# LIA-DiTella/DiffUDF

Measured on AMD Instinct MI355X. Metric: train points/sec (SIREN fwd+∇x+Eikonal loss+bwd), 256×8 net, 100k pts, higher is better.
Workload: dtype f32

## Files before the change

### diffudf_amd/csrc/dudf_api.hip

```cpp
#include "dudf_context.h"

namespace {

int split_mask() { return dudf_split_mask(dudf_options()); }

int check_ws(const DudfLayout& lo, const void* ws, size_t bytes) {
    if (int rc = dudf_check_buffer(ws, bytes, lo.total_bytes)) return rc;
    if (lo.np > (1ll << 25)) return DUDF_E_BADCFG;
    return 0;
}

SweepRequest make_request(int which, int H, const SweepArgs& a) {
    return SweepRequest{which, H, a.L, a.store_s, a.store_c, a.train, a.have_e, a.split, a.p24, a.ebound != nullptr, a.zbound != nullptr};
}

int check_loss_mode(int mode, bool backward, int64_t n_hess, const double* weights, const double* stats) {
    if (mode != DUDF_LOSS_S1 && mode != DUDF_LOSS_SIREN && !(backward && mode == DUDF_LOSS_S2)) return DUDF_E_BADMODE;
    if (mode == DUDF_LOSS_S2 && !stats) return DUDF_E_BADMODE;
    if (n_hess != 0 && !(mode == DUDF_LOSS_S1 && weights[2] != 0.0)) return DUDF_E_BADMODE;
    return 0;
}

int64_t stash_offset(const DudfLayout& lo, int which) {
    const int64_t offs[8] = {lo.ws_S, lo.ws_C, lo.ws_Q, lo.ws_E, lo.ws_A, lo.ws_Z, lo.ws_R, lo.ws_ZS};
    return offs[which];
}

}

SweepArgs dudf_make_sweep_args(const DudfLayout& lo, const float* theta, float* ws) {
    SweepArgs a;
    a.theta = theta; a.w1b = ws + lo.ws_w1b; a.b1s = ws + lo.ws_b1s; a.w1t16 = ws + lo.ws_w1t16; a.wt = ws + lo.ws_wt;
    a.wimg_f = reinterpret_cast<const char*>(ws + lo.ws_wimg);
    a.wimg_t = a.wimg_f + (size_t)(lo.L - 1) * lo.H * lo.H * 6;
    a.wimg16_f = reinterpret_cast<const char*>(ws + lo.ws_wimg16);
    a.wimg16_t = a.wimg16_f + (size_t)(lo.L - 1) * lo.H * lo.H * 4;
    a.wsc = ws + lo.ws_wsc;
    a.amax = reinterpret_cast<unsigned*>(ws + lo.ws_amax);
    a.ebound = (lo.ws_ebound != lo.ws_amax) ? ws + lo.ws_ebound : nullptr;
    a.zbound = (lo.ws_zbound != lo.ws_amax) ? ws + lo.ws_zbound : nullptr;
    a.nch = lo.ncol_h;
    a.split = split_mask();
    a.clk = nullptr;
    a.x4 = ws + lo.ws_x4; a.y = ws + lo.ws_y; a.g = ws + lo.ws_g; a.ybar = ws + lo.ws_ybar; a.gbar = ws + lo.ws_gbar;
    a.S = ws + lo.ws_S; a.C = ws + lo.ws_C; a.ZS = ws + lo.ws_ZS; a.Q = ws + lo.ws_Q; a.R = ws + lo.ws_R;
    a.E = ws + lo.ws_E; a.A = ws + lo.ws_A; a.Z = ws + lo.ws_Z;
    a.np = lo.np; a.stash_layer = lo.stash_layer;
    a.off_hid = lo.off_hid; a.hid_stride = lo.hid_stride; a.off_wo = lo.off_wo; a.off_bo = lo.off_bo;
    a.L = lo.L; a.w0 = lo.w0;
    a.store_s = 0; a.store_c = 0; a.train = 0; a.have_e = 1;
    a.tile0 = 0; a.ntiles = 0; a.hess = 0;
    a.p24 = lo.p24;
    a.fxs = nullptr;
    return a;
}

int dudf_launch_range(int which, int H, SweepArgs a, hipStream_t st) {
    const SweepChoice c = dudf_choose_sweep(make_request(which, H, a), dudf_options());
    if (c.status) return c.status;
    DudfProfScope prof(PROF_SWEEP_FWD + (which & 3), st);
    if (which <= SWEEP_ADJ_REV) dudf_note_products(PROF_SWEEP_FWD + which, c.products);
    a.store_s = c.store_s; a.store_c = c.store_c;
    if (c.family == DUDF_FAM_F32) return dudf_launch_sweep(c, a, st);
    if (which <= SWEEP_ADJ_REV) a.clk = dudf_prof_clk(PROF_SWEEP_FWD + which);
    return dudf_launch_sweep_bf16(c, a, st);
}

int dudf_run_sweep(int base, const DudfLayout& lo, SweepArgs a, hipStream_t st) {
    int rc = 0;
    if ((lo.p24 & 1) && base >= SWEEP_FWD && base <= SWEEP_ADJ_REV) a.fxs = a.S - lo.ws_S + lo.ws_fx[base];
    SweepArgs aq = a, ap = a;
    aq.tile0 = 0; aq.ntiles = (int)(lo.ncol_h / DUDF_TILE_PTS); aq.hess = 1;
    ap.tile0 = aq.ntiles; ap.ntiles = (int)(lo.ncol_n / DUDF_TILE_PTS); ap.hess = 0;
    if (lo.ncol_h > 0 && lo.ncol_n > 0) {
        const SweepChoice c = dudf_choose_pair(make_request(base, lo.H, a), dudf_options());
        if (c.status == 0) {
            DudfProfScope prof(PROF_SWEEP_FWD + base, st);
            dudf_note_products(PROF_SWEEP_FWD + base, c.products);
            ap.clk = dudf_prof_clk(PROF_SWEEP_FWD + base);
            return dudf_launch_sweep_pair(c, aq, ap, st);
        }
    }
    if (lo.ncol_h > 0 && (rc = dudf_launch_range(base + 4, lo.H, aq, st))) return rc;
    if (lo.ncol_n > 0 && (rc = dudf_launch_range(base, lo.H, ap, st))) return rc;
    return 0;
}

int dudf_open_ctx(const dudf_net_cfg* cfg, int64_t n, int64_t n_h, void* workspace, size_t bytes, void* stream, DudfCtx* c,
                  int query_only) {
    int rc = dudf_make_layout(cfg, n, n_h, &c->lo, query_only);
    if (rc) return rc;
    if ((rc = check_ws(c->lo, workspace, bytes))) return rc;
    c->st = reinterpret_cast<hipStream_t>(stream);
    c->ws = reinterpret_cast<float*>(workspace);
    return 0;
}

int dudf_forward_common(DudfCtx& c, const float* theta, const float* x, int train, bool reverse) {
    int rc;
    const DudfLayout& lo = c.lo;
    const bool all16 = train && lo.ncol_h == 0 && dudf_use_bf16_sweeps() && (split_mask() & 15) == 15 && lo.L <= 32;
    const int need = (all16 ? 0 : 1) | (!dudf_use_bf16_sweeps() ? 2 : 0);
    rc = (lo.L >= 2) ? dudf_launch_prep(lo, theta, x, c.ws, need, c.st) : DUDF_E_UNSUPPORTED;
    if (rc == DUDF_E_UNSUPPORTED) {
        if ((rc = dudf_launch_pack(c.lo, theta, c.ws, c.st))) return rc;
        if (dudf_use_bf16_sweeps() && (rc = dudf_launch_pack_bf16(c.lo, theta, c.ws, c.st))) return rc;
        if (x && (rc = dudf_launch_make_x4(c.lo, x, c.ws, c.st))) return rc;
        hipError_t e = hipMemsetAsync(c.ws + c.lo.ws_acc, 0, (size_t)2 * DUDF_NACC * sizeof(float), c.st);
        if (e == hipSuccess) e = hipMemsetAsync(c.ws + c.lo.ws_amax, 0, (size_t)4 * c.lo.L * sizeof(unsigned), c.st);
        if (e != hipSuccess) return (int)e;
    } else if (rc) {
        return rc;
    }
    SweepArgs a = dudf_make_sweep_args(c.lo, theta, c.ws);
    a.store_s = train ? 1 : 0; a.store_c = (reverse || train) ? 1 : 0; a.train = train;
    if ((rc = dudf_run_sweep(SWEEP_FWD, c.lo, a, c.st))) return rc;
    if (reverse && (rc = dudf_run_sweep(SWEEP_REV, c.lo, a, c.st))) return rc;
    return 0;
}

int dudf_backward_common(DudfCtx& c, const float* theta, int have_g, float* dtheta, int accumulate, bool zeroed) {
    int rc;
    if (!accumulate && !zeroed) {
        hipError_t e = hipMemsetAsync(dtheta, 0, (size_t)c.lo.n_theta * sizeof(float), c.st);
        if (e != hipSuccess) return (int)e;
    }
    if ((rc = dudf_backward_sweeps(c, theta, have_g, zeroed))) return rc;
    return dudf_launch_wgrad(c.lo, c.ws, dtheta, have_g, c.st);
}

int dudf_backward_sweeps(DudfCtx& c, const float* theta, int have_g, bool zeroed) {
    int rc;
    SweepArgs a = dudf_make_sweep_args(c.lo, theta, c.ws);
    a.train = 1;
    if (dudf_split_fp16() && !(zeroed && 2 * c.lo.L <= 256)) {
        hipError_t e = hipMemsetAsync(c.ws + c.lo.ws_amax + c.lo.L, 0, (size_t)2 * c.lo.L * sizeof(unsigned), c.st);
        if (e != hipSuccess) return (int)e;
    }
    if (have_g) {
        if ((rc = dudf_run_sweep(SWEEP_ADJ_FWD, c.lo, a, c.st))) return rc;
    } else {
        a.have_e = 0;
    }
    return dudf_run_sweep(SWEEP_ADJ_REV, c.lo, a, c.st);
}

extern "C" {

int dudf_sweeps_bf16x6(const dudf_net_cfg* cfg) {
    if (!cfg) return 0;
    const SweepRequest r = {SWEEP_FWD, cfg->hidden, cfg->n_hidden_layers, 0, 0, 0, 1, split_mask(), 0, false, false};
    const SweepChoice c = dudf_choose_sweep(r, dudf_options());
    return (c.status == 0 && c.family != DUDF_FAM_F32) ? 1 : 0;
}

int64_t dudf_theta_count(const dudf_net_cfg* cfg) {
    DudfLayout lo;
    if (dudf_make_layout(cfg, 1, 0, &lo)) return -1;
    return lo.n_theta;
}

size_t dudf_workspace_bytes(const dudf_net_cfg* cfg, int64_t n) { return dudf_workspace_bytes_hess(cfg, n, 0); }

size_t dudf_workspace_bytes_query(const dudf_net_cfg* cfg, int64_t n, int64_t n_hess) {
    DudfLayout lo;
    if (dudf_make_layout(cfg, n, n_hess, &lo, 1)) return 0;
    return lo.total_bytes;
}

size_t dudf_workspace_bytes_hess(const dudf_net_cfg* cfg, int64_t n, int64_t n_hess) {
    DudfLayout lo;
    if (dudf_make_layout(cfg, n, n_hess, &lo)) return 0;
    return lo.total_bytes;
}

int dudf_stash_mode(const dudf_net_cfg* cfg, int64_t n, int64_t n_hess) {
    DudfLayout lo;
    if (dudf_make_layout(cfg, n, n_hess, &lo)) return -1;
    return lo.p24;
}

int dudf_loss_forward(const dudf_net_cfg* cfg, int mode, const float* theta, const float* x, const float* normals,
                      const float* sdf, int64_t n_local, int64_t n_global, int64_t n_hess, const double* weights,
                      double alpha, float* out_terms, void* workspace, size_t workspace_bytes, void* stream) {
    int rc = check_loss_mode(mode, false, n_hess, weights, nullptr);
    if (rc) return rc;
    DudfCtx c;
    if ((rc = dudf_open_ctx(cfg, n_local, n_hess, workspace, workspace_bytes, stream, &c))) return rc;
    if ((rc = dudf_forward_common(c, theta, x, 1, true))) return rc;
    return dudf_launch_loss_fwd(c.lo, mode, normals, sdf, n_global, weights, alpha, c.ws, out_terms, c.st);
}
// ... 154 lines not shown
```

### diffudf_amd/csrc/dudf_internal.h

```cpp
#pragma once
#include <hip/hip_runtime.h>
#include <stdint.h>
#include <stdlib.h>
#include "../../include/dudf_hip.h"
#include "dudf_variants.h"

typedef float f32x4 __attribute__((ext_vector_type(4)));
typedef float f32x16 __attribute__((ext_vector_type(16)));
typedef float f32x2 __attribute__((ext_vector_type(2)));
typedef unsigned u32x4 __attribute__((ext_vector_type(4)));
typedef __bf16 bf16x8 __attribute__((ext_vector_type(8)));
typedef __bf16 bf16x2 __attribute__((ext_vector_type(2)));
typedef _Float16 f16x8 __attribute__((ext_vector_type(8)));
typedef _Float16 f16x2 __attribute__((ext_vector_type(2)));

__device__ __forceinline__ unsigned cvt_pk(f32x2 v) {
    return __builtin_bit_cast(unsigned, __builtin_convertvector(v, bf16x2));
}
__device__ __forceinline__ f32x2 unpack(unsigned p) {
    return f32x2{__builtin_bit_cast(float, p << 16), __builtin_bit_cast(float, p & 0xffff0000u)};
}

#define DUDF_TILE_PTS 64
#define DUDF_COL_PAD 128
#define DUDF_NACC 16

struct DudfLayout {
    int H, L;
    float rho;
    int p24;
    float w0;
    int64_t n, n_h;
    int64_t ncol_h, ncol_n;
    int64_t ncols;
    int64_t np;
    int64_t off_w1, off_b1, off_hid, hid_stride, off_wo, off_bo, n_theta;
    int64_t ws_w1b, ws_b1s, ws_w1t16, ws_wt, ws_wimg, ws_wimg16, ws_wsc, ws_amax, ws_ebound, ws_zbound, ws_x4, ws_y, ws_g, ws_ybar, ws_gbar;
    int64_t ws_S, ws_C, ws_ZS, ws_Q, ws_R, ws_E, ws_A, ws_Z, ws_acc;
    int64_t ws_fx[4];
    int64_t stash_layer;
    size_t total_bytes;
};

DudfOptions dudf_options();
inline bool dudf_deterministic() { return dudf_options().deterministic != 0; }
inline bool dudf_split_fp16() { return dudf_options().split != 0; }
inline int dudf_wgrad_max_workgroups() { return dudf_options().wgrad_max_workgroups; }

struct DudfCarver { int64_t o; int64_t take(int64_t cnt) { const int64_t r = o; o += (cnt + 63) / 64 * 64; return r; } };

inline int dudf_grid_for(int64_t n, int block, int cap) {
    int64_t g = (n + block - 1) / block;
    if (g < 1) g = 1;
    if (g > cap) g = cap;
    return (int)g;
}

inline size_t dudf_round256(size_t b) { return (b + 255) / 256 * 256; }

static inline int dudf_make_layout(const dudf_net_cfg* cfg, int64_t n, int64_t n_h, DudfLayout* lo, int query_only = 0) {
    if (!cfg || cfg->n_in != 3 || cfg->n_hidden_layers < 1) return DUDF_E_BADCFG;
    const int H = cfg->hidden, L = cfg->n_hidden_layers;
    if (!(H == 32 || H == 64 || H == 128 || H == 256 || H == 512)) return DUDF_E_BADCFG;
    if (n < 0 || n_h < 0 || n_h > n) return DUDF_E_BADCFG;
    if (!(cfg->w0 > 0.f) || cfg->ww < 0.f) return DUDF_E_BADCFG;
    const float ww = cfg->ww > 0.f ? cfg->ww : cfg->w0;
    lo->H = H; lo->L = L; lo->w0 = ww; lo->rho = cfg->w0 / ww;
    lo->n = n; lo->n_h = n_h;
    lo->p24 = query_only ? 0 : dudf_stash_p24_enabled(H, L, dudf_options());
    auto pad = [](int64_t c) { return (c + DUDF_COL_PAD - 1) / DUDF_COL_PAD * DUDF_COL_PAD; };
    lo->ncol_h = pad(4 * n_h);
    lo->ncol_n = pad(n - n_h);
    lo->np = lo->ncol_h + lo->ncol_n;
    if (lo->np == 0) { lo->ncol_n = DUDF_COL_PAD; lo->np = DUDF_COL_PAD; }
    lo->ncols = lo->np;
    if (lo->np % 2048 == 0) lo->np += 32;
    if (lo->np * 1024 >= (1ll << 32)) lo->p24 = 0;
    lo->off_w1 = 0; lo->off_b1 = 3 * (int64_t)H;
    lo->off_hid = 4 * (int64_t)H; lo->hid_stride = (int64_t)H * H + H;
    lo->off_wo = lo->off_hid + (L - 1) * lo->hid_stride; lo->off_bo = lo->off_wo + H;
    lo->n_theta = lo->off_bo + 1;
    DudfCarver cv = {0};
    lo->ws_w1b = cv.take(4 * (int64_t)H);
    lo->ws_b1s = cv.take((int64_t)L * H);
    lo->ws_w1t16 = cv.take(16 * (int64_t)H);
    lo->ws_wt = cv.take((int64_t)(L - 1) * H * H);
    lo->ws_wimg = cv.take((int64_t)(L - 1) * H * H * 3);
    lo->ws_wimg16 = cv.take((int64_t)(L - 1) * H * H * 2);
    lo->ws_wsc = cv.take(2 * (int64_t)(L > 1 ? L - 1 : 1));
    lo->ws_amax = cv.take(4 * (int64_t)L);
    lo->ws_ebound = query_only ? lo->ws_amax : cv.take((int64_t)L * lo->np);
    lo->ws_zbound = (n_h == 0) ? lo->ws_amax : cv.take((int64_t)L * lo->ncol_h);
    lo->ws_x4 = cv.take(4 * lo->np);
    lo->ws_y = cv.take(lo->np); lo->ws_g = cv.take(4 * lo->np);
    lo->ws_ybar = cv.take(lo->np); lo->ws_gbar = cv.take(4 * lo->np);
    lo->stash_layer = (int64_t)H * lo->np;
    const int64_t stash = (int64_t)L * lo->stash_layer;
    const int64_t stash_b = (lo->p24 & 1) ? stash / 4 * 3 : stash;
    const int64_t stash_r = (lo->p24 & 2) ? stash / 4 * 3 : stash;
    const int64_t stash_c = (lo->p24 & 4) ? stash / 4 * 3 : stash;
    lo->ws_S = cv.take(stash_b); lo->ws_C = cv.take(stash_c);
    lo->ws_ZS = n_h > 0 ? cv.take(stash) : lo->ws_S;
    if (query_only) {
        lo->ws_Q = lo->ws_R = lo->ws_E = lo->ws_A = lo->ws_Z = lo->ws_S;
    } else {
        lo->ws_Q = cv.take(stash_b); lo->ws_R = cv.take(stash_r); lo->ws_E = cv.take(stash_r); lo->ws_A = cv.take(stash_b);
        lo->ws_Z = cv.take(stash_b);
    }
    for (int i = 0; i < 4; ++i) lo->ws_fx[i] = (lo->p24 & 1) ? cv.take((int64_t)L * lo->np) : lo->ws_amax;
    lo->ws_acc = cv.take(2 * DUDF_NACC);
    lo->total_bytes = (size_t)cv.o * sizeof(float);
    return 0;
}

#if defined(__HIP_DEVICE_COMPILE__)
#define DUDF_NO_PK __attribute__((target("no-packed-fp32-ops")))
#else
#define DUDF_NO_PK
#endif

struct SweepArgs {
    const float* theta; const float* w1b; const float* b1s; const float* w1t16; const float* wt;
    const char* wimg_f; const char* wimg_t;
    const char* wimg16_f; const char* wimg16_t;
    const float* wsc;
    unsigned* amax;
    float* ebound;
    float* zbound;
    int64_t nch;
    unsigned long long* clk;
    int split;
    const float* x4;
    float* y; float* g;
    const float* ybar; const float* gbar;
    float *S, *C, *ZS, *Q, *R, *E, *A, *Z;
    int64_t np, stash_layer;
    int tile0, ntiles;
    int hess;
    int64_t off_hid, hid_stride, off_wo, off_bo;
    int L; float w0;
    int store_s, store_c, train;
    int have_e;
    int p24;
    float* fxs;
};

template <auto Kernel, class... Args>
int dudf_launch_kernel(dim3 grid, dim3 block, size_t lds, size_t lds_max, hipStream_t st, const Args&... args) {
    static bool attr_done = false;
    if (!attr_done) {
        hipError_t e = hipFuncSetAttribute(reinterpret_cast<const void*>(Kernel), hipFuncAttributeMaxDynamicSharedMemorySize, (int)lds_max);
        if (e != hipSuccess) return (int)e;
        attr_done = true;
    }
    hipLaunchKernelGGL(Kernel, grid, block, lds, st, args...);
    return (int)hipGetLastError();
}

int dudf_launch_sweep(const SweepChoice& c, const SweepArgs& a, hipStream_t st);
int dudf_launch_sweep_bf16(const SweepChoice& c, const SweepArgs& a, hipStream_t st);
int dudf_launch_sweep_wide(const SweepChoice& c, const SweepArgs& a, hipStream_t st);
int dudf_launch_sweep_pair(const SweepChoice& c, const SweepArgs& aq, const SweepArgs& ap, hipStream_t st);
int dudf_launch_pack_bf16(const DudfLayout& lo, const float* theta, float* ws, hipStream_t st);

int dudf_launch_pack(const DudfLayout& lo, const float* theta, float* ws, hipStream_t st);
int dudf_launch_wgrad(const DudfLayout& lo, float* ws, float* dtheta, int have_g, hipStream_t st, int layer_begin = 0,
                      int layer_end = 1 << 30);
int dudf_launch_make_x4(const DudfLayout& lo, const float* x, float* ws, hipStream_t st);
int dudf_launch_field_features(const DudfLayout& lo, const float* ws, int inverse_mode, double alpha, float* out_df,
                               float* out_vec, int* out_flag_count, float* out_lam, float* out_V, hipStream_t st);
int dudf_launch_loss_fwd(const DudfLayout& lo, int mode, const float* normals, const float* sdf, int64_t n_global,
                         const double* w, double alpha, float* ws, float* out_terms, hipStream_t st);
int dudf_launch_loss_bwd(const DudfLayout& lo, int mode, const float* normals, const float* sdf, int64_t n_global,
                         const double* w, double alpha, const float* cot, const double* stats, float* ws,
                         hipStream_t st, float* zero_f = nullptr, int64_t zero_fn = 0);
int dudf_launch_prep(const DudfLayout& lo, const float* theta, const float* x, float* ws, int need, hipStream_t st);
int dudf_launch_s2_stats(const DudfLayout& lo, const float* sdf, float* ws, double* stats, hipStream_t st);
int dudf_launch_s2_terms(const double* stats, const double* w, float* out_terms, hipStream_t st);
void dudf_adam_factors(double lr, double b1, double b2, int64_t step, float* step_size, float* bc2_sqrt);
int dudf_launch_adam_sched(float* theta, const float* g, float* m, float* v, int64_t n, double b1, double b2, double eps,
                           const float* sched, int64_t n_rows, const int64_t* row, double gscale, hipStream_t st);
int dudf_launch_adam(float* theta, const float* g, float* m, float* v, int64_t n, double lr, double b1, double b2,
                     double eps, int64_t step, double gscale, hipStream_t st);
int dudf_launch_read_stash(const DudfLayout& lo, const float* src, int layer, int channel, float* out, hipStream_t st, int per_quad = 0, int p24 = 0,
                           const float* fx = nullptr);
int dudf_launch_copy_in(const DudfLayout& lo, const float* ybar, const float* gbar, float* ws, hipStream_t st);
int dudf_launch_copy_out(const DudfLayout& lo, const float* ws, float* out_f, float* out_g, float* out_h,
                         hipStream_t st);
int dudf_launch_rays_x4(const DudfLayout& lo, const double* t0, float* ws, hipStream_t st);
int64_t dudf_pc_tiles(int64_t n);
int dudf_launch_pc_append(const unsigned char* flags, int64_t n, const double* src_a, const double* src_b, const float* src_f,
                          double* dst_a, double* dst_b, float* out_f, int* rows, int64_t capacity, int64_t quota, int64_t* counter,
                          int* scratch, hipStream_t st);
// ... 14 lines not shown
```

### diffudf_amd/csrc/dudf_prep.hip

```cpp
#include "dudf_sweep16.h"

namespace {

template <int H>
__device__ __forceinline__ void pack_bf16_body(const float* __restrict__ theta, char* __restrict__ img_f,
                                               char* __restrict__ img_t, int nhid, int64_t off_hid,
                                               int64_t hid_stride, int64_t block, int64_t nblocks) {
    using G = GeoB<H>;
    const int64_t total = (int64_t)2 * nhid * G::NKB * G::NT * 64;
    for (int64_t idx = block * 256 + threadIdx.x; idx < total; idx += nblocks * 256) {
        int64_t v = idx;
        const int lane = (int)(v & 63); v >>= 6;
        const int T = (int)(v % G::NT); v /= G::NT;
        const int kb = (int)(v % G::NKB); v /= G::NKB;
        const int j = (int)(v % nhid); v /= nhid;
        const int dir = (int)v;
        const int m = lane & 15, g = lane >> 4;
        const int row = 16 * T + m;
        const float* W = theta + off_hid + (int64_t)j * hid_stride;
        f32x4 e0, e1;
#pragma unroll
        for (int e = 0; e < 4; ++e) {
            const int f0 = 32 * kb + 4 * g + e, f1 = f0 + 16;
            e0[e] = dir == 0 ? W[(int64_t)row * H + f0] : W[(int64_t)f0 * H + row];
// ... 82 lines not shown
    int b = blockIdx.x;
    const int nhid = a.L - 1;
    if (b < a.nb_f16) { pack_f16_body<H>(a.theta, a.img16_f, a.img16_t, a.wsc, nhid, a.off_hid, a.hid_stride, b / a.nsub, b % a.nsub, a.nsub); return; }
    b -= a.nb_f16;
    if (b < a.nb_bf16) { pack_bf16_body<H>(a.theta, a.img_f, a.img_t, nhid, a.off_hid, a.hid_stride, b, a.nb_bf16); return; }
    b -= a.nb_bf16;
    if (b < a.nb_x4) {
        for (int64_t c = (int64_t)b * 256 + threadIdx.x; c < a.np; c += (int64_t)a.nb_x4 * 256) {
            f32x4 v = {0, 0, 0, 0};
            if (c < a.ncol_h) {
                const int64_t p = c >> 2; const int ch = (int)(c & 3);
                if (p < a.n_h) {
                    if (ch == 0) v = f32x4{a.x[p * 3], a.x[p * 3 + 1], a.x[p * 3 + 2], 1.f};
                    else v[ch - 1] = 1.f;
                }
            } else {
                const int64_t p = a.n_h + (c - a.ncol_h);
                if (p < a.n) v = f32x4{a.x[p * 3], a.x[p * 3 + 1], a.x[p * 3 + 2], 1.f};
            }
            *reinterpret_cast<f32x4*>(a.x4 + c * 4) = v;
        }
        return;
    }
    b -= a.nb_x4;
    if (b < a.nb_thin) {
        const int n_thin = 16 * H > a.L * H ? 16 * H : a.L * H;
        for (int gid = b * 256 + threadIdx.x; gid < n_thin; gid += a.nb_thin * 256) {
            if (gid < 4 * H) {
                const int f = gid / 4, k = gid % 4;
                a.w1b[gid] = a.rho * (k < 3 ? a.theta[f * 3 + k] : a.theta[3 * H + f]);
                if (k == 3) a.b1s[f] = a.rho * a.theta[3 * H + f];
            }
            if (gid >= H && gid < a.L * H) {
                const int layer = gid / H, f = gid % H;
                a.b1s[gid] = a.theta[a.off_hid + (int64_t)(layer - 1) * a.hid_stride + (int64_t)H * H + f];
            }
            if (gid < 16 * H) {
                const int r = gid / H, f = gid % H;
                a.w1t16[gid] = r < 3 ? a.rho * a.theta[f * 3 + r] : 0.f;
            }
        }
        if (b == 0) {
            for (int i = threadIdx.x; i < a.nzero; i += 256) a.zero[i] = 0u;
            for (int i = threadIdx.x; i < a.nzero2; i += 256) a.zero2[i] = 0u;
        }
        return;
    }
    b -= a.nb_thin;
    {
        const int64_t n_wt = (int64_t)nhid * H * H;
        for (int64_t gid = (int64_t)b * 256 + threadIdx.x; gid < n_wt; gid += (int64_t)a.nb_wt * 256) {
            const int64_t j = gid / ((int64_t)H * H), rem = gid % ((int64_t)H * H);
            const int i = (int)(rem / H), o = (int)(rem % H);
            a.wt[gid] = a.theta[a.off_hid + j * a.hid_stride + (int64_t)o * H + i];
        }
    }
}

template <int H>
int pack_b(const DudfLayout& lo, const float* theta, float* ws, hipStream_t st) {
    using G = GeoB<H>;
    char* img_f = reinterpret_cast<char*>(ws + lo.ws_wimg);
    char* img_t = img_f + (size_t)(lo.L - 1) * G::IMGB;
    const int64_t total = (int64_t)2 * (lo.L - 1) * G::NKB * G::NT * 64;
    hipLaunchKernelGGL(pack_bf16_kernel<H>, dim3((unsigned)((total + 255) / 256)), dim3(256), 0, st, theta, img_f, img_t,
                       lo.L - 1, lo.off_hid, lo.hid_stride);
    if (dudf_split_fp16()) {
        using G1 = GeoB<H, 1>;
        char* i16_f = reinterpret_cast<char*>(ws + lo.ws_wimg16);
        char* i16_t = i16_f + (size_t)(lo.L - 1) * G1::IMGB;
        hipLaunchKernelGGL(pack_f16_kernel<H>, dim3(H >= 256 ? 16 : 4, lo.L - 1), dim3(256), 0, st, theta, i16_f, i16_t,
                           ws + lo.ws_wsc, lo.L - 1, lo.off_hid, lo.hid_stride);
    }
    return (int)hipGetLastError();
}

template <int H>
int prep_b(const DudfLayout& lo, const float* theta, const float* x, float* ws, int need, hipStream_t st) {
    PrepArgs a;
    a.theta = theta; a.x = x;
    a.w1b = ws + lo.ws_w1b; a.b1s = ws + lo.ws_b1s; a.rho = lo.rho; a.w1t16 = ws + lo.ws_w1t16; a.wt = ws + lo.ws_wt; a.x4 = ws + lo.ws_x4; a.wsc = ws + lo.ws_wsc;
    a.img_f = reinterpret_cast<char*>(ws + lo.ws_wimg); a.img_t = a.img_f + (size_t)(lo.L - 1) * GeoB<H>::IMGB;
    a.img16_f = reinterpret_cast<char*>(ws + lo.ws_wimg16); a.img16_t = a.img16_f + (size_t)(lo.L - 1) * GeoB<H, 1>::IMGB;
    a.zero = reinterpret_cast<unsigned*>(ws + lo.ws_acc); a.nzero = 2 * DUDF_NACC;
    a.zero2 = reinterpret_cast<unsigned*>(ws + lo.ws_amax); a.nzero2 = 4 * lo.L;
    a.L = lo.L; a.off_hid = lo.off_hid; a.hid_stride = lo.hid_stride;
    a.n = lo.n; a.n_h = lo.n_h; a.ncol_h = lo.ncol_h; a.np = lo.np;
    const int nhid = lo.L - 1;
    a.nsub = H >= 256 ? 16 : 4;
    a.nb_f16 = (dudf_split_fp16() && nhid > 0) ? nhid * a.nsub : 0;
    a.nb_bf16 = ((need & 1) && nhid > 0) ? (int)(((int64_t)2 * nhid * GeoB<H>::NKB * GeoB<H>::NT * 64 + 255) / 256) : 0;
    a.nb_x4 = x ? (int)((lo.np + 255) / 256 < 1024 ? (lo.np + 255) / 256 : 1024) : 0;
    a.nb_thin = 2;
    a.nb_wt = ((need & 2) && nhid > 0) ? (int)(((int64_t)nhid * H * H + 255) / 256 < 2048 ? ((int64_t)nhid * H * H + 255) / 256 : 2048) : 0;
    const int grid = a.nb_f16 + a.nb_bf16 + a.nb_x4 + a.nb_thin + a.nb_wt;
    hipLaunchKernelGGL(prep_kernel<H>, dim3(grid), dim3(256), 0, st, a);
    return (int)hipGetLastError();
}
}

int dudf_launch_prep(const DudfLayout& lo, const float* theta, const float* x, float* ws, int need, hipStream_t st) {
    DudfProfScope prof(PROF_PACK, st);
    if (lo.H == 256) return prep_b<256>(lo, theta, x, ws, need, st);
    if (lo.H == 128) return prep_b<128>(lo, theta, x, ws, need, st);
    if (lo.H == 512) return prep_b<512>(lo, theta, x, ws, need, st);
    return DUDF_E_UNSUPPORTED;
}

int dudf_launch_pack_bf16(const DudfLayout& lo, const float* theta, float* ws, hipStream_t st) {
    if (lo.L < 2) return 0;
    DudfProfScope prof(PROF_PACK, st);
    if (lo.H == 256) return pack_b<256>(lo, theta, ws, st);
    if (lo.H == 128) return pack_b<128>(lo, theta, ws, st);
    if (lo.H == 512) return pack_b<512>(lo, theta, ws, st);
    return 0;
}
```

### diffudf_amd/csrc/dudf_wgrad.hip

```cpp
#include "dudf_internal.h"
#include <stdlib.h>
#include <string.h>
#include <type_traits>

namespace {

template <int H> struct WG;
template <> struct WG<256> { static constexpr int WO = 4, WI = 2, MT = 2, NTL = 4; };
template <> struct WG<128> { static constexpr int WO = 4, WI = 2, MT = 1, NTL = 2; };
template <> struct WG<64>  { static constexpr int WO = 2, WI = 2, MT = 1, NTL = 1; };
template <> struct WG<32>  { static constexpr int WO = 1, WI = 1, MT = 1, NTL = 1; };

constexpr int KT = 32;
constexpr int KTP = 33;

struct WgradArgs {
    const float *Q, *A, *Z, *S;
    int64_t ncol_h;
    float* dtheta;
    int64_t np, stash_layer, off_hid, hid_stride;
    int steps_total;
    int L;
    int have_g;
    int j0, nj;
// ... 724 lines not shown
    drain();
    using B0 = std::integral_constant<int, 0>; using B1 = std::integral_constant<int, 1>; using B2 = std::integral_constant<int, 2>;
    for (; it < nhot; it += 3) {
        stage(it, R2, std::true_type{}, B0{});
        stage(it + 1, R0, std::true_type{}, B1{});
        stage(it + 2, R1, std::true_type{}, B2{});
    }
    drain();
    for (; it < nit; it += 3) {
        stage(it, R2, std::false_type{}, B0{});
        if (it + 1 < nit) stage(it + 1, R0, std::false_type{}, B1{});
        if (it + 2 < nit) stage(it + 2, R1, std::false_type{}, B2{});
    }
#if DUDF_WGRAD_DBG & 32
    if (bx == 3 && by == 10 && lane == 0)
        for (int i = 0; i < 12; ++i) g_wstamp[wave][i] = wst[i];
#endif

    float* dW = a.dtheta + a.off_hid + (int64_t)j * a.hid_stride + (int64_t)o_off * a.Hs + i_off;
    float* dB = a.dtheta + a.off_hid + (int64_t)j * a.hid_stride + (int64_t)a.Hs * a.Hs + o_off;
    if (nit > 0) {
        const int l32 = lane & 31, hh = lane >> 5;
#pragma unroll
        for (int m = 0; m < W::MT; ++m)
#pragma unroll
            for (int e = 0; e < 16; ++e) {
                const int o = (wo * W::MT + m) * 32 + (e & 3) + 8 * (e >> 2) + 4 * hh;
#pragma unroll
                for (int n = 0; n < W::NTL; ++n) {
                    const int i = (wi * W::NTL + n) * 32 + l32;
#if DUDF_WGRAD_DBG & 64
                    asm volatile("" :: "v"(acc[m][n][e]));
#else
                    atomicAdd(dW + (int64_t)o * a.Hs + i, SP != 0 ? acc[m][n][e] * inv_p : acc[m][n][e]);
#endif
                }
            }
        if (p_oper == 0 && i_off == 0) {
            if constexpr (P24 != 0) {
                const float bun = P24 == 1 ? 1.0f / sc1 : 1.0f;
                auto red = [&](float v, int f) {
                    v += __shfl_xor(v, 1); v += __shfl_xor(v, 2); v += __shfl_xor(v, 4); v += __shfl_xor(v, 8);
                    if (p_li == 0) atomicAdd(dB + f, v * bun);
                };
                const f32x4 bs[4] = {bacc, bacc1, bacc2, bacc3};
#pragma unroll
                for (int t = 0; t < 4; ++t)
#pragma unroll
                    for (int e = 0; e < 4; ++e) red(bs[t][e], 16 * (4 * pw + t) + 4 * p_q + e);
            } else {
            auto red = [&](float v, int f) {
                v += __shfl_xor(v, 1);
                v += __shfl_xor(v, 2);
                if (p_cg == 0) atomicAdd(dB + 4 * p_fq + f, v);
            };
            red(bacc.x, 0); red(bacc.y, 1); red(bacc.z, 2); red(bacc.w, 3);
            }
        }
    }
    if (clk_on && tid == 0) {
        a.clk[0] = __builtin_amdgcn_s_memtime() - clk_t0;
        a.clk[1] = __builtin_amdgcn_s_memrealtime() - clk_r0;
    }
}
template <int VAR> constexpr int wg_buffers() { static_assert(VAR == 9 || VAR == 25, "VAR 9: three image buffers, 25: four"); return VAR == 25 ? 4 : 3; }
template <int H, int VAR>
__global__ __launch_bounds__(64 * WG<H>::WO * WG<H>::WI) DUDF_NO_PK void wgrad_hidden_bf16p_kernel(WgradArgs a) {
    wgrad_hidden_bf16p_body<H, wg_buffers<VAR>()>(a);
}
template <int H, int VAR>
__global__ __launch_bounds__(64 * WG<H>::WO * WG<H>::WI) DUDF_NO_PK void wgrad_hidden_f16p_kernel(WgradArgs a) {
    wgrad_hidden_bf16p_body<H, wg_buffers<VAR>(), 1>(a);
}
template <int H, int VAR>
__global__ __launch_bounds__(64 * WG<H>::WO * WG<H>::WI) DUDF_NO_PK void wgrad_hidden_f16tr_kernel(WgradArgs a) {
    wgrad_hidden_bf16p_body<H, wg_buffers<VAR>(), 1, 2>(a);
}
template <int H, int VAR>
__global__ __launch_bounds__(64 * WG<H>::WO * WG<H>::WI) DUDF_NO_PK void wgrad_hidden_f16p24_kernel(WgradArgs a) {
    wgrad_hidden_bf16p_body<H, wg_buffers<VAR>(), 1, 1>(a);
}

#ifndef DUDF_WGSMALL_P24_PTS
#define DUDF_WGSMALL_P24_PTS 4096
#endif
struct WgradSmallArgs {
    const float *Q, *A, *Z, *S;
    const float *x4, *gbar, *ybar;
    float* dtheta;
    int64_t np, ncols, stash_layer, off_wo, off_bo;
    int H, L, have_g;
    int pts_per_block;
    float rho;
    const float *fxS, *fxQ, *fxA, *fxZ;
};

__device__ __forceinline__ float wave_sum(float v) {
#pragma unroll
    for (int o = 32; o > 0; o >>= 1) v += __shfl_xor(v, o);
    return v;
}

__device__ __forceinline__ void wgrad_small_body(const WgradSmallArgs& a) {
    const int lane = threadIdx.x & 63, wave = threadIdx.x >> 6;
    const int FQ = a.H / 4;
    const int64_t p0 = (int64_t)blockIdx.x * a.pts_per_block;
    const int64_t p1 = (p0 + a.pts_per_block < a.ncols) ? p0 + a.pts_per_block : a.ncols;
    const float* Q0 = a.Q;
    const float* Z0 = a.Z;
    const float* AL = a.A + (int64_t)(a.L - 1) * a.stash_layer;
    const float* SL = a.S + (int64_t)(a.L - 1) * a.stash_layer;
    const int fq_per = (FQ + gridDim.y - 1) / gridDim.y;
    const int fq_lo = blockIdx.y * fq_per, fq_hi = (fq_lo + fq_per < FQ) ? fq_lo + fq_per : FQ;
    for (int fq = fq_lo + wave; fq < fq_hi; fq += 4) {
        float w1[4][4], wo[4];
#pragma unroll
        for (int c = 0; c < 4; ++c) { wo[c] = 0.f; w1[c][0] = w1[c][1] = w1[c][2] = w1[c][3] = 0.f; }
#pragma unroll 4
        for (int64_t p = p0 + lane; p < p1; p += 64) {
            const int64_t off = ((int64_t)fq * a.np + p) * 4;
            const f32x4 z = __builtin_nontemporal_load(reinterpret_cast<const f32x4*>(Z0 + off));
            const f32x4 sl = __builtin_nontemporal_load(reinterpret_cast<const f32x4*>(SL + off));
            const f32x4 xv = *reinterpret_cast<const f32x4*>(a.x4 + p * 4);
            const float yb = a.ybar[p];
            f32x4 qv = {0, 0, 0, 0}, al = {0, 0, 0, 0}, gb = {0, 0, 0, 0};
            if (a.have_g) {
                qv = __builtin_nontemporal_load(reinterpret_cast<const f32x4*>(Q0 + off));
                al = __builtin_nontemporal_load(reinterpret_cast<const f32x4*>(AL + off));
                gb = *reinterpret_cast<const f32x4*>(a.gbar + p * 4);
            }
#pragma unroll
            for (int c = 0; c < 4; ++c) {
#pragma unroll
                for (int d = 0; d < 4; ++d) w1[c][d] += qv[c] * gb[d] + z[c] * xv[d];
                wo[c] += al[c] * xv[3] + yb * sl[c];
            }
        }
#pragma unroll
        for (int c = 0; c < 4; ++c) {
            const int f = 4 * fq + c;
#pragma unroll
            for (int d = 0; d < 4; ++d) {
                const float v = wave_sum(w1[c][d]);
                if (lane == 0) atomicAdd(d < 3 ? a.dtheta + f * 3 + d : a.dtheta + 3 * a.H + f, a.rho * v);
            }
            const float vo = wave_sum(wo[c]);
            if (lane == 0) atomicAdd(a.dtheta + a.off_wo + f, vo);
        }
    }
    if (wave == 0 && blockIdx.y == 0) {
        float s = 0.f;
        for (int64_t p = p0 + lane; p < p1; p += 64) s += a.ybar[p];
        s = wave_sum(s);
        if (lane == 0) atomicAdd(a.dtheta + a.off_bo, s);
    }
}
__global__ __launch_bounds__(256) DUDF_NO_PK void wgrad_small_kernel(WgradSmallArgs a) { wgrad_small_body(a); }

__device__ __forceinline__ f32x4 small_unpack24(const unsigned* g, const float sc) {
    typedef unsigned u3_t __attribute__((ext_vector_type(3)));
    const u3_t d = __builtin_nontemporal_load(reinterpret_cast<const u3_t*>(g));
    const unsigned d0 = d.x, d1 = d.y, d2 = d.z;
    const unsigned m = 0x00ffffffu, two = 0x40000000u;
    const unsigned y = __builtin_amdgcn_perm(d1, d0, 0x0c0c0703u);
    const unsigned t3 = __builtin_amdgcn_perm(d2, y, 0x0c070100u) | two;
    const float m3 = -3.0f * sc;
    return f32x4{__builtin_fmaf(__uint_as_float((d0 & m) | two), sc, m3), __builtin_fmaf(__uint_as_float((d1 & m) | two), sc, m3),
                 __builtin_fmaf(__uint_as_float((d2 & m) | two), sc, m3), __builtin_fmaf(__uint_as_float(t3), sc, m3)};
}
__global__ __launch_bounds__(256) DUDF_NO_PK void wgrad_small_p24_kernel(WgradSmallArgs a) {
    const int lane = threadIdx.x & 63, wave = threadIdx.x >> 6;
    const int q = lane >> 4, li = lane & 15, T = blockIdx.y;
    const int64_t ng = a.np >> 4;
    const int64_t g0 = (int64_t)blockIdx.x * (a.pts_per_block >> 4);
    const int64_t gend = (a.ncols + 15) >> 4;
    const int64_t g1 = g0 + (a.pts_per_block >> 4) < gend ? g0 + (a.pts_per_block >> 4) : gend;
    const int64_t lbytes = a.stash_layer * 3;
    auto tile = [&](const float* arr, int layer) { return reinterpret_cast<const char*>(arr) + (int64_t)layer * lbytes + (int64_t)T * ng * 768 + lane * 12; };
    const char* Q0 = tile(a.Q, 0); const char* Z0 = tile(a.Z, 0);
    const char* AL = tile(a.A, a.L - 1); const char* SL = tile(a.S, a.L - 1);
    float w1[4][4], wo[4];
#pragma unroll
    for (int c = 0; c < 4; ++c) { wo[c] = 0.f; w1[c][0] = w1[c][1] = w1[c][2] = w1[c][3] = 0.f; }
    float sy = 0.f;
    const int nwave = (int)(blockDim.x >> 6);
#pragma unroll 4
    for (int64_t g = g0 + wave; g < g1; g += nwave) {
        const int64_t p = g * 16 + li;
        const f32x4 z = small_unpack24(reinterpret_cast<const unsigned*>(Z0 + g * 768), a.fxZ[p]);
        const f32x4 sl = small_unpack24(reinterpret_cast<const unsigned*>(SL + g * 768), a.fxS[(int64_t)(a.L - 1) * a.np + p]);
        const f32x4 xv = *reinterpret_cast<const f32x4*>(a.x4 + p * 4);
        const float yb = a.ybar[p];
        f32x4 qv = {0, 0, 0, 0}, al = {0, 0, 0, 0}, gb = {0, 0, 0, 0};
        if (a.have_g) {
            qv = small_unpack24(reinterpret_cast<const unsigned*>(Q0 + g * 768), a.fxQ[p]);
            al = small_unpack24(reinterpret_cast<const unsigned*>(AL + g * 768), a.fxA[(int64_t)(a.L - 1) * a.np + p]);
            gb = *reinterpret_cast<const f32x4*>(a.gbar + p * 4);
        }
        sy += yb;
#pragma unroll
        for (int c = 0; c < 4; ++c) {
#pragma unroll
            for (int d = 0; d < 4; ++d) w1[c][d] += qv[c] * gb[d] + z[c] * xv[d];
            wo[c] += al[c] * xv[3] + yb * sl[c];
        }
    }
    auto sum16 = [](float v) { v += __shfl_xor(v, 1); v += __shfl_xor(v, 2); v += __shfl_xor(v, 4); v += __shfl_xor(v, 8); return v; };
    __shared__ float red[4][4][21];
#pragma unroll
    for (int c = 0; c < 4; ++c) {
#pragma unroll
        for (int d = 0; d < 4; ++d) {
            const float v = sum16(w1[c][d]);
            if (li == 0) red[wave][q][c * 4 + d] = v;
        }
        const float vo = sum16(wo[c]);
        if (li == 0) red[wave][q][16 + c] = vo;
    }
    {
        const float v = sum16(sy);
        if (li == 0) red[wave][q][20] = v;
    }
    __syncthreads();
    for (int t = threadIdx.x; t < 81; t += blockDim.x) {
        if (t < 80) {
            const int qq = t / 20, k = t % 20;
            float v = 0.f;
            for (int w = 0; w < nwave; ++w) v += red[w][qq][k];
            if (k < 16) {
                const int c = k >> 2, d = k & 3, f = 16 * T + 4 * qq + c;
                atomicAdd(d < 3 ? a.dtheta + f * 3 + d : a.dtheta + 3 * a.H + f, a.rho * v);
            } else {
                atomicAdd(a.dtheta + a.off_wo + 16 * T + 4 * qq + (k - 16), v);
            }
        } else if (T == 0) {
            float v = 0.f;
            for (int w = 0; w < nwave; ++w) v += red[w][0][20];
            atomicAdd(a.dtheta + a.off_bo, v);
        }
    }
}

static_assert(KTP == 33 && NRING == 4 && KB == 16, "dudf_choose_wgrad: LDS sizes");
template <int H>
int launch_hidden(const SweepChoice& c, const WgradArgs& a, hipStream_t st) {
    using W = WG<H>;
    const int tz = a.Hs / H, ntz = tz * tz;
    int nsplit = dudf_wgrad_max_workgroups() / (a.nj * ntz);
    if (nsplit > a.steps_total) nsplit = a.steps_total;
    if (nsplit < 1 || dudf_deterministic()) nsplit = 1;
    const dim3 grid(a.nj, nsplit, ntz), block(64 * W::WO * W::WI);
    if (c.family == DUDF_FAM_WG_F32) return dudf_launch_kernel<&wgrad_hidden_kernel<H>>(grid, block, c.lds, c.lds_max, st, a);
    if (c.family == DUDF_FAM_WG_BF16) return dudf_launch_kernel<&wgrad_hidden_bf16_kernel<H>>(grid, block, c.lds, c.lds_max, st, a);
    if constexpr (H == 256) {
        if (c.family == DUDF_FAM_WG_F16P24 && c.fl == 25) return dudf_launch_kernel<&wgrad_hidden_f16p24_kernel<H, 25>>(grid, block, c.lds, c.lds_max, st, a);
        if (c.family == DUDF_FAM_WG_F16P24) return dudf_launch_kernel<&wgrad_hidden_f16p24_kernel<H, 9>>(grid, block, c.lds, c.lds_max, st, a);
        if (c.family == DUDF_FAM_WG_F16TR) return dudf_launch_kernel<&wgrad_hidden_f16tr_kernel<H, 9>>(grid, block, c.lds, c.lds_max, st, a);
        if (c.family == DUDF_FAM_WG_BF16P) return dudf_launch_kernel<&wgrad_hidden_bf16p_kernel<H, 9>>(grid, block, c.lds, c.lds_max, st, a);
        if (c.family == DUDF_FAM_WG_F16P && c.remap) {
            WgradArgs b = a;
            b.remap_nsplit = nsplit;
            return dudf_launch_kernel<&wgrad_hidden_f16p_kernel<H, 9>>(dim3(((a.nj * nsplit + 7) / 8) * 32), block, c.lds, c.lds_max, st, b);
        }
        if (c.family == DUDF_FAM_WG_F16P) return dudf_launch_kernel<&wgrad_hidden_f16p_kernel<H, 9>>(grid, block, c.lds, c.lds_max, st, a);
    }
    return DUDF_E_UNSUPPORTED;
}

}

int dudf_launch_wgrad(const DudfLayout& lo, float* ws, float* dtheta, int have_g, hipStream_t st, int layer_begin,
                      int layer_end) {
    if (layer_begin < 0) layer_begin = 0;
    if (layer_end > lo.L + 1) layer_end = lo.L + 1;
    WgradArgs a;
    a.Q = ws + lo.ws_Q; a.A = ws + lo.ws_A; a.Z = ws + lo.ws_Z; a.S = ws + lo.ws_S; a.ncol_h = lo.ncol_h;
    a.dtheta = dtheta; a.np = lo.np; a.stash_layer = lo.stash_layer;
    a.off_hid = lo.off_hid; a.hid_stride = lo.hid_stride; a.steps_total = (int)(lo.ncols / KT); a.L = lo.L;
    a.have_g = have_g; a.Hs = lo.H;
    a.amax = reinterpret_cast<const unsigned*>(ws + lo.ws_amax);
    a.clk = dudf_prof_clk(PROF_WGRAD_HIDDEN);
    a.remap_nsplit = 0;
    a.p24 = lo.p24 & 1;
    a.fxS = ws + lo.ws_fx[0]; a.fxQ = ws + lo.ws_fx[1]; a.fxA = ws + lo.ws_fx[2]; a.fxZ = ws + lo.ws_fx[3];
    const int hb = layer_begin < 1 ? 1 : layer_begin, he = layer_end > lo.L ? lo.L : layer_end;
    a.j0 = hb - 1; a.nj = he > hb ? he - hb : 0;
    int rc = 0;
    if (a.nj > 0) {
        DudfProfScope prof(PROF_WGRAD_HIDDEN, st);
        const SweepChoice c = dudf_choose_wgrad(WgradRequest{lo.H, lo.L, a.p24, lo.np}, dudf_options());
        if (c.status) return c.status;
        dudf_note_products(PROF_WGRAD_HIDDEN, c.products);
        switch (c.H) {
            case 32: rc = launch_hidden<32>(c, a, st); break;
            case 64: rc = launch_hidden<64>(c, a, st); break;
            case 128: rc = launch_hidden<128>(c, a, st); break;
            default: rc = launch_hidden<256>(c, a, st); break;
        }
    }
    if (rc) return rc;
    if (!(layer_begin <= 0 || layer_end >= lo.L + 1)) return 0;
    WgradSmallArgs s;
    s.Q = a.Q; s.A = a.A; s.Z = a.Z; s.S = a.S; s.x4 = ws + lo.ws_x4; s.gbar = ws + lo.ws_gbar; s.ybar = ws + lo.ws_ybar;
    s.dtheta = dtheta; s.np = lo.np; s.ncols = lo.ncols; s.stash_layer = lo.stash_layer;
    s.off_wo = lo.off_wo; s.off_bo = lo.off_bo; s.H = lo.H; s.L = lo.L; s.have_g = have_g; s.rho = lo.rho;
    s.fxS = a.fxS; s.fxQ = a.fxQ; s.fxA = a.fxA; s.fxZ = a.fxZ;
    s.pts_per_block = dudf_deterministic() ? (int)lo.ncols : 4096;
    const int grid = (int)((lo.ncols + s.pts_per_block - 1) / s.pts_per_block);
    DudfProfScope prof(PROF_WGRAD_SMALL, st);
    const int fqn = lo.H / 4;
    const int gy = fqn >= 64 ? 16 : (fqn >= 4 ? fqn / 4 : 1);
    if (lo.p24 & 1) {
        if (!dudf_deterministic()) {
            s.pts_per_block = DUDF_WGSMALL_P24_PTS;
            const int64_t want = (lo.ncols / 30 + 255) / 256 * 256;
            if (want < s.pts_per_block) s.pts_per_block = want < 512 ? 512 : (int)want;
        }
        s.pts_per_block = (s.pts_per_block + 15) / 16 * 16;
        hipLaunchKernelGGL(wgrad_small_p24_kernel, dim3((unsigned)((lo.ncols + s.pts_per_block - 1) / s.pts_per_block), lo.H / 16),
                           dim3(dudf_deterministic() ? 64 : 256), 0, st, s);
        return (int)hipGetLastError();
    }
    hipLaunchKernelGGL(wgrad_small_kernel, dim3(grid, gy), dim3(256), 0, st, s);
    return (int)hipGetLastError();
}
```

Baseline: 39.51 million.

## Replace per-block atomics in p24 small wgrad with ticketed last-block reduction

The 24-bit-packed small weight-gradient kernel now writes each block's partial sums to a workspace buffer. A per-tile ticket counter elects the last block, which reduces all partials and issues a single set of atomics into dtheta, instead of every block doing atomicAdds. Blocks shrink to 1024 points, giving more blocks and more parallelism, and the streaming loop moves to 32-bit offsets with the have_g branch hoisted into a template. The change adds workspace for the partials and tickets and drops the deterministic small-block path. Its correctness depends on the ticket reset and on memory ordering between the partial stores and the final read.

```diff
diff --git a/diffudf_amd/csrc/dudf_api.hip b/diffudf_amd/csrc/dudf_api.hip
--- a/diffudf_amd/csrc/dudf_api.hip
+++ b/diffudf_amd/csrc/dudf_api.hip
@@ -106,7 +106,7 @@
         if ((rc = dudf_launch_pack(c.lo, theta, c.ws, c.st))) return rc;
         if (dudf_use_bf16_sweeps() && (rc = dudf_launch_pack_bf16(c.lo, theta, c.ws, c.st))) return rc;
         if (x && (rc = dudf_launch_make_x4(c.lo, x, c.ws, c.st))) return rc;
-        hipError_t e = hipMemsetAsync(c.ws + c.lo.ws_acc, 0, (size_t)2 * DUDF_NACC * sizeof(float), c.st);
+        hipError_t e = hipMemsetAsync(c.ws + c.lo.ws_acc, 0, (size_t)(2 * DUDF_NACC + DUDF_NTICKET) * sizeof(float), c.st);
         if (e == hipSuccess) e = hipMemsetAsync(c.ws + c.lo.ws_amax, 0, (size_t)4 * c.lo.L * sizeof(unsigned), c.st);
         if (e != hipSuccess) return (int)e;
     } else if (rc) {
diff --git a/diffudf_amd/csrc/dudf_internal.h b/diffudf_amd/csrc/dudf_internal.h
--- a/diffudf_amd/csrc/dudf_internal.h
+++ b/diffudf_amd/csrc/dudf_internal.h
@@ -24,6 +24,9 @@
 #define DUDF_TILE_PTS 64
 #define DUDF_COL_PAD 128
 #define DUDF_NACC 16
+#define DUDF_NTICKET 32
+#define DUDF_THIN_MIN_PTS 512
+#define DUDF_THIN_SUMS 84
 
 struct DudfLayout {
     int H, L;
@@ -36,7 +39,7 @@
     int64_t np;
     int64_t off_w1, off_b1, off_hid, hid_stride, off_wo, off_bo, n_theta;
     int64_t ws_w1b, ws_b1s, ws_w1t16, ws_wt, ws_wimg, ws_wimg16, ws_wsc, ws_amax, ws_ebound, ws_zbound, ws_x4, ws_y, ws_g, ws_ybar, ws_gbar;
-    int64_t ws_S, ws_C, ws_ZS, ws_Q, ws_R, ws_E, ws_A, ws_Z, ws_acc;
+    int64_t ws_S, ws_C, ws_ZS, ws_Q, ws_R, ws_E, ws_A, ws_Z, ws_acc, ws_thin;
     int64_t ws_fx[4];
     int64_t stash_layer;
     size_t total_bytes;
@@ -108,7 +111,8 @@
         lo->ws_Z = cv.take(stash_b);
     }
     for (int i = 0; i < 4; ++i) lo->ws_fx[i] = (lo->p24 & 1) ? cv.take((int64_t)L * lo->np) : lo->ws_amax;
-    lo->ws_acc = cv.take(2 * DUDF_NACC);
+    lo->ws_acc = cv.take(2 * DUDF_NACC + DUDF_NTICKET);
+    lo->ws_thin = (lo->p24 & 1) ? cv.take((lo->ncols + DUDF_THIN_MIN_PTS - 1) / DUDF_THIN_MIN_PTS * (H / 16) * DUDF_THIN_SUMS) : lo->ws_amax;
     lo->total_bytes = (size_t)cv.o * sizeof(float);
     return 0;
 }
diff --git a/diffudf_amd/csrc/dudf_prep.hip b/diffudf_amd/csrc/dudf_prep.hip
--- a/diffudf_amd/csrc/dudf_prep.hip
+++ b/diffudf_amd/csrc/dudf_prep.hip
@@ -188,7 +188,7 @@
     a.w1b = ws + lo.ws_w1b; a.b1s = ws + lo.ws_b1s; a.rho = lo.rho; a.w1t16 = ws + lo.ws_w1t16; a.wt = ws + lo.ws_wt; a.x4 = ws + lo.ws_x4; a.wsc = ws + lo.ws_wsc;
     a.img_f = reinterpret_cast<char*>(ws + lo.ws_wimg); a.img_t = a.img_f + (size_t)(lo.L - 1) * GeoB<H>::IMGB;
     a.img16_f = reinterpret_cast<char*>(ws + lo.ws_wimg16); a.img16_t = a.img16_f + (size_t)(lo.L - 1) * GeoB<H, 1>::IMGB;
-    a.zero = reinterpret_cast<unsigned*>(ws + lo.ws_acc); a.nzero = 2 * DUDF_NACC;
+    a.zero = reinterpret_cast<unsigned*>(ws + lo.ws_acc); a.nzero = 2 * DUDF_NACC + DUDF_NTICKET;
     a.zero2 = reinterpret_cast<unsigned*>(ws + lo.ws_amax); a.nzero2 = 4 * lo.L;
     a.L = lo.L; a.off_hid = lo.off_hid; a.hid_stride = lo.hid_stride;
     a.n = lo.n; a.n_h = lo.n_h; a.ncol_h = lo.ncol_h; a.np = lo.np;
diff --git a/diffudf_amd/csrc/dudf_wgrad.hip b/diffudf_amd/csrc/dudf_wgrad.hip
--- a/diffudf_amd/csrc/dudf_wgrad.hip
+++ b/diffudf_amd/csrc/dudf_wgrad.hip
@@ -830,8 +830,9 @@
 }
 
 #ifndef DUDF_WGSMALL_P24_PTS
-#define DUDF_WGSMALL_P24_PTS 4096
+#define DUDF_WGSMALL_P24_PTS 1024
 #endif
+static_assert(DUDF_WGSMALL_P24_PTS % 16 == 0 && DUDF_WGSMALL_P24_PTS >= DUDF_THIN_MIN_PTS, "ws_thin is sized for blocks of at least DUDF_THIN_MIN_PTS columns");
 struct WgradSmallArgs {
     const float *Q, *A, *Z, *S;
     const float *x4, *gbar, *ybar;
@@ -841,6 +842,8 @@
     int pts_per_block;
     float rho;
     const float *fxS, *fxQ, *fxA, *fxZ;
+    float* part;
+    unsigned* tickets;
 };
 
 __device__ __forceinline__ float wave_sum(float v) {
@@ -905,7 +908,8 @@
 }
 __global__ __launch_bounds__(256) DUDF_NO_PK void wgrad_small_kernel(WgradSmallArgs a) { wgrad_small_body(a); }
 
-__device__ __forceinline__ f32x4 small_unpack24(const unsigned* g, const float sc) {
+constexpr int kThinSums = DUDF_THIN_SUMS;
+__device__ __forceinline__ f32x4 small_unpack24(const char* g, const float sc) {
     typedef unsigned u3_t __attribute__((ext_vector_type(3)));
     const u3_t d = __builtin_nontemporal_load(reinterpret_cast<const u3_t*>(g));
     const unsigned d0 = d.x, d1 = d.y, d2 = d.z;
@@ -916,74 +920,109 @@
     return f32x4{__builtin_fmaf(__uint_as_float((d0 & m) | two), sc, m3), __builtin_fmaf(__uint_as_float((d1 & m) | two), sc, m3),
                  __builtin_fmaf(__uint_as_float((d2 & m) | two), sc, m3), __builtin_fmaf(__uint_as_float(t3), sc, m3)};
 }
-__global__ __launch_bounds__(256) DUDF_NO_PK void wgrad_small_p24_kernel(WgradSmallArgs a) {
-    const int lane = threadIdx.x & 63, wave = threadIdx.x >> 6;
+struct ThinSums { float w[4][4], o[4], sy; };
+template <bool G>
+__device__ __forceinline__ void thin_stream_p24(const WgradSmallArgs& a, int T, int wave, int lane, ThinSums& r) {
+    const int li = lane & 15;
+    const unsigned ng = (unsigned)(a.np >> 4), gpb = (unsigned)a.pts_per_block >> 4;
+    const unsigned gend = (unsigned)((a.ncols + 15) >> 4);
+    const unsigned g0 = blockIdx.x * gpb, g1 = g0 + gpb < gend ? g0 + gpb : gend;
+    const int64_t tile_b = (int64_t)T * ng * 768, last_b = (int64_t)(a.L - 1) * a.stash_layer * 3;
+    const char* Qb = reinterpret_cast<const char*>(a.Q) + tile_b;
+    const char* Zb = reinterpret_cast<const char*>(a.Z) + tile_b;
+    const char* Ab = reinterpret_cast<const char*>(a.A) + last_b + tile_b;
+    const char* Sb = reinterpret_cast<const char*>(a.S) + last_b + tile_b;
+    const char* fQ = reinterpret_cast<const char*>(a.fxQ);
+    const char* fZ = reinterpret_cast<const char*>(a.fxZ);
+    const char* fA = reinterpret_cast<const char*>(a.fxA + (int64_t)(a.L - 1) * a.np);
+    const char* fS = reinterpret_cast<const char*>(a.fxS + (int64_t)(a.L - 1) * a.np);
+    const char* x4b = reinterpret_cast<const char*>(a.x4);
+    const char* gbb = reinterpret_cast<const char*>(a.gbar);
+    const char* ybb = reinterpret_cast<const char*>(a.ybar);
+    unsigned vs = (g0 + wave) * 768u + lane * 12u;
+    unsigned vc = ((g0 + wave) * 16u + li) * 4u;
+#pragma unroll 1
+    for (unsigned g = g0 + wave; g < g1; g += 4, vs += 4 * 768u, vc += 4 * 64u) {
+        const f32x4 z = small_unpack24(Zb + vs, *reinterpret_cast<const float*>(fZ + vc));
+        const f32x4 sl = small_unpack24(Sb + vs, *reinterpret_cast<const float*>(fS + vc));
+        const f32x4 xv = *reinterpret_cast<const f32x4*>(x4b + 4u * vc);
+        const float yb = *reinterpret_cast<const float*>(ybb + vc);
+        f32x4 qv = {0, 0, 0, 0}, al = {0, 0, 0, 0}, gb = {0, 0, 0, 0};
+        if constexpr (G) {
+            qv = small_unpack24(Qb + vs, *reinterpret_cast<const float*>(fQ + vc));
+            al = small_unpack24(Ab + vs, *reinterpret_cast<const float*>(fA + vc));
+            gb = *reinterpret_cast<const f32x4*>(gbb + 4u * vc);
+        }
+        r.sy += yb;
+#pragma unroll
+        for (int c = 0; c < 4; ++c) {
+#pragma unroll
+            for (int d = 0; d < 4; ++d) r.w[c][d] += G ? qv[c] * gb[d] + z[c] * xv[d] : z[c] * xv[d];
+            r.o[c] += G ? al[c] * xv[3] + yb * sl[c] : yb * sl[c];
+        }
+    }
+}
+__global__ __launch_bounds__(256, 8) void wgrad_small_p24_kernel(WgradSmallArgs a) {
+    const int lane = threadIdx.x & 63, wave = __builtin_amdgcn_readfirstlane(threadIdx.x >> 6);
     const int q = lane >> 4, li = lane & 15, T = blockIdx.y;
-    const int64_t ng = a.np >> 4;
-    const int64_t g0 = (int64_t)blockIdx.x * (a.pts_per_block >> 4);
-    const int64_t gend = (a.ncols + 15) >> 4;
-    const int64_t g1 = g0 + (a.pts_per_block >> 4) < gend ? g0 + (a.pts_per_block >> 4) : gend;
-    const int64_t lbytes = a.stash_layer * 3;
-    auto tile = [&](const float* arr, int layer) { return reinterpret_cast<const char*>(arr) + (int64_t)layer * lbytes + (int64_t)T * ng * 768 + lane * 12; };
-    const char* Q0 = tile(a.Q, 0); const char* Z0 = tile(a.Z, 0);
-    const char* AL = tile(a.A, a.L - 1); const char* SL = tile(a.S, a.L - 1);
-    float w1[4][4], wo[4];
-#pragma unroll
-    for (int c = 0; c < 4; ++c) { wo[c] = 0.f; w1[c][0] = w1[c][1] = w1[c][2] = w1[c][3] = 0.f; }
-    float sy = 0.f;
-    const int nwave = (int)(blockDim.x >> 6);
-#pragma unroll 4
-    for (int64_t g = g0 + wave; g < g1; g += nwave) {
-        const int64_t p = g * 16 + li;
-        const f32x4 z = small_unpack24(reinterpret_cast<const unsigned*>(Z0 + g * 768), a.fxZ[p]);
-        const f32x4 sl = small_unpack24(reinterpret_cast<const unsigned*>(SL + g * 768), a.fxS[(int64_t)(a.L - 1) * a.np + p]);
-        const f32x4 xv = *reinterpret_cast<const f32x4*>(a.x4 + p * 4);
-        const float yb = a.ybar[p];
-        f32x4 qv = {0, 0, 0, 0}, al = {0, 0, 0, 0}, gb = {0, 0, 0, 0};
-        if (a.have_g) {
-            qv = small_unpack24(reinterpret_cast<const unsigned*>(Q0 + g * 768), a.fxQ[p]);
-            al = small_unpack24(reinterpret_cast<const unsigned*>(AL + g * 768), a.fxA[(int64_t)(a.L - 1) * a.np + p]);
-            gb = *reinterpret_cast<const f32x4*>(a.gbar + p * 4);
-        }
-        sy += yb;
-#pragma unroll
-        for (int c = 0; c < 4; ++c) {
-#pragma unroll
-            for (int d = 0; d < 4; ++d) w1[c][d] += qv[c] * gb[d] + z[c] * xv[d];
-            wo[c] += al[c] * xv[3] + yb * sl[c];
-        }
-    }
+    ThinSums r = {};
+    if (a.have_g) thin_stream_p24<true>(a, T, wave, lane, r);
+    else thin_stream_p24<false>(a, T, wave, lane, r);
     auto sum16 = [](float v) { v += __shfl_xor(v, 1); v += __shfl_xor(v, 2); v += __shfl_xor(v, 4); v += __shfl_xor(v, 8); return v; };
-    __shared__ float red[4][4][21];
-#pragma unroll
-    for (int c = 0; c < 4; ++c) {
-#pragma unroll
-        for (int d = 0; d < 4; ++d) {
-            const float v = sum16(w1[c][d]);
-            if (li == 0) red[wave][q][c * 4 + d] = v;
-        }
-        const float vo = sum16(wo[c]);
-        if (li == 0) red[wave][q][16 + c] = vo;
-    }
+    __shared__ float red[4 * kThinSums];
     {
-        const float v = sum16(sy);
-        if (li == 0) red[wave][q][20] = v;
+        float* dst = red + wave * kThinSums + q * 21;
+        float v[21];
+#pragma unroll
+        for (int k = 0; k < 16; ++k) v[k] = sum16(r.w[k >> 2][k & 3]);
+#pragma unroll
+        for (int k = 0; k < 4; ++k) v[16 + k] = sum16(r.o[k]);
+        v[20] = sum16(r.sy);
+        if (li == 0) {
+#pragma unroll
+            for (int k = 0; k < 21; ++k) dst[k] = v[k];
+        }
     }
     __syncthreads();
-    for (int t = threadIdx.x; t < 81; t += blockDim.x) {
-        if (t < 80) {
-            const int qq = t / 20, k = t % 20;
-            float v = 0.f;
-            for (int w = 0; w < nwave; ++w) v += red[w][qq][k];
-            if (k < 16) {
-                const int c = k >> 2, d = k & 3, f = 16 * T + 4 * qq + c;
-                atomicAdd(d < 3 ? a.dtheta + f * 3 + d : a.dtheta + 3 * a.H + f, a.rho * v);
-            } else {
-                atomicAdd(a.dtheta + a.off_wo + 16 * T + 4 * qq + (k - 16), v);
-            }
-        } else if (T == 0) {
-            float v = 0.f;
-            for (int w = 0; w < nwave; ++w) v += red[w][0][20];
+    const int tid = threadIdx.x;
+    const unsigned nbx = gridDim.x;
+    float* part = a.part + (size_t)T * nbx * kThinSums;
+    if (tid < kThinSums)
+        __hip_atomic_store(part + (size_t)blockIdx.x * kThinSums + tid,
+                           (red[tid] + red[kThinSums + tid]) + (red[2 * kThinSums + tid] + red[3 * kThinSums + tid]), __ATOMIC_RELAXED,
+                           __HIP_MEMORY_SCOPE_AGENT);
+    asm volatile("s_waitcnt vmcnt(0)" ::: "memory");
+    __syncthreads();
+    if (tid == 0) {
+        const bool last = __hip_atomic_fetch_add(a.tickets + T, 1u, __ATOMIC_RELAXED, __HIP_MEMORY_SCOPE_AGENT) == nbx - 1;
+        if (last) {
+            __builtin_amdgcn_fence(__ATOMIC_ACQUIRE, "agent");
+            asm volatile("s_waitcnt vmcnt(0)" ::: "memory");
+            __hip_atomic_store(a.tickets + T, 0u, __ATOMIC_RELAXED, __HIP_MEMORY_SCOPE_AGENT);
+        }
+        red[0] = last ? 1.f : 0.f;
+    }
+    __syncthreads();
+    if (red[0] == 0.f) return;
+    __syncthreads();
+    if (tid < 3 * kThinSums) {
+        const unsigned third = tid / kThinSums, b0 = nbx * third / 3, b1 = nbx * (third + 1) / 3;
+        const float* src = part + (tid - third * kThinSums);
+        float v = 0.f;
+#pragma unroll 8
+        for (unsigned b = b0; b < b1; ++b) v += src[(size_t)b * kThinSums];
+        red[tid] = v;
+    }
+    __syncthreads();
+    if (tid < kThinSums) {
+        const float v = (red[tid] + red[kThinSums + tid]) + red[2 * kThinSums + tid];
+        const int qq = tid / 21, k = tid % 21, f = 16 * T + 4 * qq;
+        if (k < 16) {
+            const int c = k >> 2, d = k & 3;
+            atomicAdd(d < 3 ? a.dtheta + (f + c) * 3 + d : a.dtheta + 3 * a.H + f + c, a.rho * v);
+        } else if (k < 20) {
+            atomicAdd(a.dtheta + a.off_wo + f + (k - 16), v);
+        } else if (T == 0 && qq == 0) {
             atomicAdd(a.dtheta + a.off_bo, v);
         }
     }
@@ -1052,21 +1091,19 @@
     s.Q = a.Q; s.A = a.A; s.Z = a.Z; s.S = a.S; s.x4 = ws + lo.ws_x4; s.gbar = ws + lo.ws_gbar; s.ybar = ws + lo.ws_ybar;
     s.dtheta = dtheta; s.np = lo.np; s.ncols = lo.ncols; s.stash_layer = lo.stash_layer;
     s.off_wo = lo.off_wo; s.off_bo = lo.off_bo; s.H = lo.H; s.L = lo.L; s.have_g = have_g; s.rho = lo.rho;
-    s.fxS = a.fxS; s.fxQ = a.fxQ; s.fxA = a.fxA; s.fxZ = a.fxZ;
+    s.fxS = a.fxS; s.fxQ = a.fxQ; s.fxA = a.fxA; s.fxZ = a.fxZ; s.part = nullptr; s.tickets = nullptr;
     s.pts_per_block = dudf_deterministic() ? (int)lo.ncols : 4096;
     const int grid = (int)((lo.ncols + s.pts_per_block - 1) / s.pts_per_block);
     DudfProfScope prof(PROF_WGRAD_SMALL, st);
     const int fqn = lo.H / 4;
     const int gy = fqn >= 64 ? 16 : (fqn >= 4 ? fqn / 4 : 1);
     if (lo.p24 & 1) {
-        if (!dudf_deterministic()) {
-            s.pts_per_block = DUDF_WGSMALL_P24_PTS;
-            const int64_t want = (lo.ncols / 30 + 255) / 256 * 256;
-            if (want < s.pts_per_block) s.pts_per_block = want < 512 ? 512 : (int)want;
-        }
-        s.pts_per_block = (s.pts_per_block + 15) / 16 * 16;
+        s.pts_per_block = DUDF_WGSMALL_P24_PTS;
+        s.part = ws + lo.ws_thin;
+        s.tickets = reinterpret_cast<unsigned*>(ws + lo.ws_acc) + 2 * DUDF_NACC;
+        if (lo.H / 16 > DUDF_NTICKET) return DUDF_E_UNSUPPORTED;
         hipLaunchKernelGGL(wgrad_small_p24_kernel, dim3((unsigned)((lo.ncols + s.pts_per_block - 1) / s.pts_per_block), lo.H / 16),
-                           dim3(dudf_deterministic() ? 64 : 256), 0, st, s);
+                           dim3(256), 0, st, s);
         return (int)hipGetLastError();
     }
     hipLaunchKernelGGL(wgrad_small_kernel, dim3(grid, gy), dim3(256), 0, st, s);
```

Result: no change. 39.71 million, median of 6 (+0.5%).
